# openfheorg/openfhe-boolean-circuit-evaluator

Hardware: AMD Instinct MI355X
Metric: encrypted gate-bootstraps/sec (whole node), AES-128 Bristol ckt STD128 GINX (higher is better)
Workload: dtype u32

## Files before the change

openfhe-boolean-circuit-evaluator_amd/csrc/kernels.hip:

```cpp
#include <hip/hip_runtime.h>

#include <algorithm>
#include <utility>

#include "kernels.hpp"

namespace bce {

#include "phase_prof.hpp"
#include "fused_tail.hpp"
#include "dag_sched.hpp"
#ifdef BCE_PHASE_PROF
__device__ unsigned long long g_phase_prof[BCE_PROF_WAVES * BCE_PROF_SLOTS];
#define BCE_PROF_ARRAY ::bce::g_phase_prof
#endif

__device__ __forceinline__ u32 csub(u32 x, u32 m) { return min(x, x - m); }

__device__ __forceinline__ u32 mul_shoup_lazy(u32 y, uint2 w, u32 Q) {
    u32 qh = __umulhi(w.y, y);
    return w.x * y - qh * Q;
}

__device__ __forceinline__ u64 mad64(u32 a, u32 b, u64 c) {
    u64 r, carry;
    asm("v_mad_u64_u32 %0, %1, %2, %3, %4" : "=v"(r), "=s"(carry) : "v"(a), "v"(b), "v"(c));
    return r;
}
__device__ __forceinline__ u64 mul64(u32 a, u32 b) {
    u64 r, carry;
    asm("v_mad_u64_u32 %0, %1, %2, %3, 0" : "=v"(r), "=s"(carry) : "v"(a), "v"(b));
    return r;
}
__device__ __forceinline__ u32 mul_shoup_lazy3(u32 y, uint2 w, u32 Q) {
    return (u32)mad64(__umulhi(w.y, y), 0u - Q, mul64(y, w.x));
}
__device__ __forceinline__ u64 pair_of(u32 lo) {
    u64 p;
    asm volatile("" : "=v"(p));
    return (p & 0xFFFFFFFF00000000ull) | lo;
}
__device__ __forceinline__ u64 with_lo(u64 pair, u32 lo) { return (pair & 0xFFFFFFFF00000000ull) | lo; }

__device__ __forceinline__ u32 barrett_lazy3(u64 x, u32 Q, u32 shift, u32 mu) {
    return (u32)mad64(__umulhi((u32)(x >> shift), mu), 0u - Q, x);
}

__device__ __forceinline__ u32 barrett_reduce(u64 x, u32 Q, u32 shift, u32 mu) {
    u32 x1 = (u32)(x >> shift);
    u32 qh = __umulhi(x1, mu);
    u32 r = (u32)x - qh * Q;
    r = csub(r, 2 * Q);
    return csub(r, Q);
}

__device__ __forceinline__ u32 barrett_fold(u64 x, u32 c32, u32 Q, u32 shift, u32 mu) {
    return barrett_reduce((u64)(u32)(x >> 32) * c32 + (u32)x, Q, shift, mu);
}

__device__ __forceinline__ u32 phys(u32 j) { return j + ((j >> 6) << 2); }

template <int LOGN>
struct Cfg {
    static constexpr int N = 1 << LOGN;
    static constexpr int LE = LOGN - 6;
    static constexpr int E = 1 << LE;
    static constexpr int NP = N + (N >> 6) * 4;
    static constexpr int F2LO = (6 > LE) ? 6 - LE : 0;
    static_assert(LOGN >= 9 && LOGN <= 11, "supported ring sizes: 512, 1024, 2048");
};

template <u32 M>
__device__ __forceinline__ u32 tw_pos(u32 i) {
    if constexpr (M < 64) {
        return M + i;
    } else {
        constexpr u32 sh = __builtin_ctz(M) - 6;
        return M + ((i & ((1u << sh) - 1u)) << 6) + (i >> sh);
    }
}

__device__ __forceinline__ void block_sync_lds() {
    asm volatile("s_waitcnt lgkmcnt(0)\n\ts_barrier" ::: "memory");
}

__device__ __forceinline__ void wave_sync();
__device__ __forceinline__ void wave_local_sync() {
#ifdef BCE_STEP_BARRIERS
    block_sync_lds();
#else
    wave_sync();
#endif
}
__device__ __forceinline__ void wave_sync() {
    __builtin_amdgcn_fence(__ATOMIC_RELEASE, "wavefront");
    __builtin_amdgcn_wave_barrier();
    __builtin_amdgcn_fence(__ATOMIC_ACQUIRE, "wavefront");
}

template <int LOGN, int LO>
__device__ __forceinline__ u32 elem_j(u32 lane, int r) {
    constexpr int LE = Cfg<LOGN>::LE;
    u32 lane_lo = lane & ((1u << LO) - 1u);
    u32 lane_hi = lane >> LO;
    return (lane_hi << (LO + LE)) | ((u32)r << LO) | lane_lo;
}

template <int LOGN, int LO>
__device__ __forceinline__ void load_pass(const u32* poly, u32 lane, u32 (&x)[Cfg<LOGN>::E]) {
    constexpr int E = Cfg<LOGN>::E;
    if constexpr (LO == 0) {
        const uint4* p = reinterpret_cast<const uint4*>(poly + phys(lane * E));
#pragma unroll
        for (int k = 0; k < E / 4; ++k) {
            uint4 v = p[k];
            x[4 * k] = v.x; x[4 * k + 1] = v.y; x[4 * k + 2] = v.z; x[4 * k + 3] = v.w;
        }
    } else {
#pragma unroll
        for (int r = 0; r < E; ++r) x[r] = poly[phys(elem_j<LOGN, LO>(lane, r))];
    }
}

template <int LOGN, int LO>
__device__ __forceinline__ void store_pass(u32* poly, u32 lane, const u32 (&x)[Cfg<LOGN>::E]) {
    constexpr int E = Cfg<LOGN>::E;
    if constexpr (LO == 0) {
        uint4* p = reinterpret_cast<uint4*>(poly + phys(lane * E));
#pragma unroll
        for (int k = 0; k < E / 4; ++k) p[k] = make_uint4(x[4 * k], x[4 * k + 1], x[4 * k + 2], x[4 * k + 3]);
    } else {
#pragma unroll
        for (int r = 0; r < E; ++r) poly[phys(elem_j<LOGN, LO>(lane, r))] = x[r];
    }
}

template <int LOGN, int LO, int B, bool LAZY>
__device__ __forceinline__ void fwd_stage(u32 (&x)[Cfg<LOGN>::E], u32 lane, const uint2* tw, u32 Q) {
    constexpr int LE = Cfg<LOGN>::LE, E = Cfg<LOGN>::E;
    constexpr int rb = B - LO;
    constexpr u32 m = 1u << (LOGN - 1 - B);
    const u32 hi = (lane >> LO) << (LO + LE - B - 1);
    const u32 Q2 = 2 * Q;
#pragma unroll
    for (int r = 0; r < E; ++r) {
        if (r & (1 << rb)) continue;
        uint2 w = tw[tw_pos<m>(hi | (u32)(r >> (rb + 1)))];
        u32 X = LAZY ? x[r] : csub(x[r], Q2);
        u32 T = mul_shoup_lazy(x[r | (1 << rb)], w, Q);
        x[r] = X + T;
        x[r | (1 << rb)] = X + Q2 - T;
    }
}

template <int LOGN, int LO, int B>
__device__ __forceinline__ void fwd_stage_pair(u64 (&x)[Cfg<LOGN>::E], u32 lane, const uint2* tw, u32 Q) {
    constexpr int LE = Cfg<LOGN>::LE, E = Cfg<LOGN>::E;
    constexpr int rb = B - LO;
    constexpr u32 m = 1u << (LOGN - 1 - B);
    const u32 hi = (lane >> LO) << (LO + LE - B - 1);
    const u32 Q2 = 2 * Q, negQ = 0u - Q;
#pragma unroll
    for (int r = 0; r < E; ++r) {
        if (r & (1 << rb)) continue;
// ... 96 lines not shown
        constexpr int b = gs_bound(r, RB0, RBEND);
        if constexpr (b == 4) x[r] = csub(x[r], 2 * Q);
        else if constexpr (b > 4) x[r] = x[r] - __umulhi(x[r], mu32) * Q;
    };
    (red(std::integral_constant<int, R>{}), ...);
}

template <int LOGN, int LO, int BHI, int BLO, bool LAZY>
__device__ __forceinline__ void fwd_stages(u32 (&x)[Cfg<LOGN>::E], u32 lane, const uint2* tw, u32 Q) {
    if constexpr (BHI >= BLO) {
        fwd_stage<LOGN, LO, BHI, LAZY>(x, lane, tw, Q);
        fwd_stages<LOGN, LO, BHI - 1, BLO, LAZY>(x, lane, tw, Q);
    }
}
template <int LOGN, bool LAZY, bool NORM = true, bool LM_IN = false>
__device__ __forceinline__ void ntt_forward_wave(u32* poly, const uint2* twf, u32 lane, u32 Q, u32 mu32) {
    using C = Cfg<LOGN>;
    u32 x[C::E];
    if constexpr (LAZY && C::F2LO > 0) {
        u64 xp[C::E];
        if constexpr (LM_IN) {
            load_lm<LOGN>(poly, lane, x);
            fwd_first_stage_pair<LOGN>(x, xp, twf[1], Q);
            fwd_stages_pair<LOGN, 6, LOGN - 2, 6>(xp, lane, twf, Q);
        } else {
            load_pass_pair<LOGN, 6>(poly, lane, xp);
            fwd_stages_pair<LOGN, 6, LOGN - 1, 6>(xp, lane, twf, Q);
        }
        store_pass_pair<LOGN, 6>(poly, lane, xp);
        wave_sync();
        load_pass_pair<LOGN, C::F2LO>(poly, lane, xp);
        fwd_stages_pair<LOGN, C::F2LO, 5, C::F2LO>(xp, lane, twf, Q);
        store_pass_pair<LOGN, C::F2LO>(poly, lane, xp);
        wave_sync();
        load_pass<LOGN, 0>(poly, lane, x);
        fwd_stages<LOGN, 0, C::F2LO - 1, 0, LAZY>(x, lane, twf, Q);
    } else {
        if constexpr (LM_IN) load_lm<LOGN>(poly, lane, x);
        else load_pass<LOGN, 6>(poly, lane, x);
        fwd_stages<LOGN, 6, LOGN - 1, 6, LAZY>(x, lane, twf, Q);
        store_pass<LOGN, 6>(poly, lane, x);
        wave_sync();
        load_pass<LOGN, C::F2LO>(poly, lane, x);
        fwd_stages<LOGN, C::F2LO, 5, C::F2LO, LAZY>(x, lane, twf, Q);
        if constexpr (C::F2LO > 0) {
            store_pass<LOGN, C::F2LO>(poly, lane, x);
            wave_sync();
            load_pass<LOGN, 0>(poly, lane, x);
            fwd_stages<LOGN, 0, C::F2LO - 1, 0, LAZY>(x, lane, twf, Q);
        }
    }
    if constexpr (NORM || !LAZY) {
#pragma unroll
        for (int r = 0; r < C::E; ++r) {
            if constexpr (LAZY) {
                u32 v = x[r] - __umulhi(x[r], mu32) * Q;
                x[r] = csub(csub(v, 2 * Q), Q);
            } else {
                x[r] = csub(csub(x[r], 2 * Q), Q);
            }
        }
    }
    store_pass<LOGN, 0>(poly, lane, x);
    wave_sync();
}

__device__ __forceinline__ void ntt_forward_wave_low8(u32* poly, const uint2* twf, u32 lane, u32 Q) {
    constexpr int LOGN = 10;
    {
        u64 xp[16];
        load_pass_pair<LOGN, 4>(poly, lane, xp);
        fwd_stages_pair<LOGN, 4, 7, 4>(xp, lane, twf, Q);
        store_pass_pair<LOGN, 4>(poly, lane, xp);
    }
    wave_sync();
    u32 x[16];
    u64 xp[16];
    load_pass<LOGN, 0>(poly, lane, x);
    fwd_first_stage_pair<LOGN>(x, xp, twf[tw_pos<64>(lane)], Q);
    fwd_stages_pair<LOGN, 0, 2, 0>(xp, lane, twf, Q);
#pragma unroll
    for (int r = 0; r < 16; ++r) x[r] = (u32)xp[r];
    store_pass<LOGN, 0>(poly, lane, x);
    wave_sync();
}
__device__ __forceinline__ void fwd_bfly_pair(u64& xa, u64& xb, uint2 w, u32 Q) {
    const u32 X = (u32)xa, Y = (u32)xb;
    const u64 t = mad64(__umulhi(Y, w.y), 0u - Q, mad64(Y, w.x, xa));
    xb = with_lo(xb, (X << 1) + 2 * Q - (u32)t);
    xa = t;
}
__device__ __forceinline__ void ntt_forward_half_low8(u32* row, u32 h, const uint2* twf, u32 lane, u32 Q) {
    asm volatile("" : "+v"(lane));
    u64 xp[8];
    {
        const u32 l8 = lane >> 5, j0 = (h << 9) | (l8 << 8) | (lane & 31u);
        u32* const p = row + phys(j0);
#pragma unroll
        for (int r = 0; r < 8; ++r) xp[r] = pair_of(p[(r >> 1) * 68 + (r & 1) * 32]);
        const u32 i7 = (h << 1) | l8;
        const uint2 w7 = twf[tw_pos<4>(i7)];
#pragma unroll
        for (int r = 0; r < 4; ++r) fwd_bfly_pair(xp[r], xp[r + 4], w7, Q);
#pragma unroll
        for (int g = 0; g < 2; ++g) {
            const uint2 w6 = twf[tw_pos<8>((i7 << 1) | g)];
            fwd_bfly_pair(xp[4 * g], xp[4 * g + 2], w6, Q);
            fwd_bfly_pair(xp[4 * g + 1], xp[4 * g + 3], w6, Q);
        }
#pragma unroll
        for (int g = 0; g < 4; ++g) fwd_bfly_pair(xp[2 * g], xp[2 * g + 1], twf[tw_pos<16>((i7 << 2) | g)], Q);
#pragma unroll
        for (int r = 0; r < 8; ++r) p[(r >> 1) * 68 + (r & 1) * 32] = (u32)xp[r];
    }
    wave_sync();
    {
        const u32 lh = lane >> 2, j0 = (h << 9) | (lh << 5) | (lane & 3u);
        u32* const p = row + phys(j0);
#pragma unroll
        for (int r = 0; r < 8; ++r) xp[r] = pair_of(p[4 * r]);
        const u32 i4 = (h << 4) | lh;
        const uint2 w4 = twf[tw_pos<32>(i4)];
#pragma unroll
        for (int r = 0; r < 4; ++r) fwd_bfly_pair(xp[r], xp[r + 4], w4, Q);
#pragma unroll
        for (int g = 0; g < 2; ++g) {
            const uint2 w3 = twf[tw_pos<64>((i4 << 1) | g)];
            fwd_bfly_pair(xp[4 * g], xp[4 * g + 2], w3, Q);
            fwd_bfly_pair(xp[4 * g + 1], xp[4 * g + 3], w3, Q);
        }
#pragma unroll
        for (int g = 0; g < 4; ++g) fwd_bfly_pair(xp[2 * g], xp[2 * g + 1], twf[tw_pos<128>((i4 << 2) | g)], Q);
#pragma unroll
        for (int r = 0; r < 8; ++r) p[4 * r] = (u32)xp[r];
    }
    wave_sync();
    {
        const u32 j0 = (h << 9) | (lane << 3);
        uint4* const p = reinterpret_cast<uint4*>(row + phys(j0));
        const uint4 v0 = p[0], v1 = p[1];
        xp[0] = pair_of(v0.x); xp[1] = pair_of(v0.y); xp[2] = pair_of(v0.z); xp[3] = pair_of(v0.w);
        xp[4] = pair_of(v1.x); xp[5] = pair_of(v1.y); xp[6] = pair_of(v1.z); xp[7] = pair_of(v1.w);
        const u32 i1 = (((h << 6) | lane) << 1);
#pragma unroll
        for (int g = 0; g < 2; ++g) {
            const uint2 w1 = twf[tw_pos<256>(i1 | g)];
            fwd_bfly_pair(xp[4 * g], xp[4 * g + 2], w1, Q);
            fwd_bfly_pair(xp[4 * g + 1], xp[4 * g + 3], w1, Q);
        }
#pragma unroll
        for (int g = 0; g < 4; ++g) fwd_bfly_pair(xp[2 * g], xp[2 * g + 1], twf[tw_pos<512>((i1 << 1) | g)], Q);
        p[0] = make_uint4((u32)xp[0], (u32)xp[1], (u32)xp[2], (u32)xp[3]);
        p[1] = make_uint4((u32)xp[4], (u32)xp[5], (u32)xp[6], (u32)xp[7]);
    }
    wave_sync();
}
__device__ __forceinline__ void fwd_bfly(u32& X, u32& Y, uint2 w, u32 Q) {
    const u64 t = mad64(__umulhi(Y, w.y), 0u - Q, mad64(Y, w.x, pair_of(X)));
    Y = (X << 1) + 2 * Q - (u32)t;
    X = (u32)t;
}

template <int LOGN>
__device__ __forceinline__ void ntt_inverse_wave(const u32* src, u32* tmp, const uint2* twi, u32 lane, u32 Q,
                                                 uint2 ninv, uint2 wlast, u32 mu32, u32 (&x)[Cfg<LOGN>::E]) {
    using C = Cfg<LOGN>;
    constexpr int LE = C::LE;
    constexpr auto regs = std::make_integer_sequence<int, C::E>{};
    load_pass<LOGN, 0>(src, lane, x);
    inv_stages<LOGN, 0, 0, LE - 1, 0, false>(x, lane, twi, Q, ninv, wlast);
    inv_pass_reduce<LOGN, 0, LE>(x, Q, mu32, regs);
    store_pass<LOGN, 0>(tmp, lane, x);
    wave_sync();
    load_pass<LOGN, LE>(tmp, lane, x);
    inv_stages<LOGN, LE, LE, 2 * LE - 1, 0, false>(x, lane, twi, Q, ninv, wlast);
    inv_pass_reduce<LOGN, 0, LE>(x, Q, mu32, regs);
    store_pass<LOGN, LE>(tmp, lane, x);
    wave_sync();
    load_pass<LOGN, 6>(tmp, lane, x);
    inv_stages<LOGN, 6, 2 * LE, LOGN - 1, 2 * LE - 6, true>(x, lane, twi, Q, ninv, wlast);
}

template <int LOGN>
__device__ __forceinline__ u32 psi_pow(__amdgpu_buffer_rsrc_t psi_rsrc, u32 e, u32 Q) {
    constexpr u32 N = 1u << LOGN;
    const u32 v = __builtin_amdgcn_raw_buffer_load_b32(psi_rsrc, (e & (N - 1)) << 2, 0, 0);
    return (e & N) ? Q - v : v;
}

__device__ __forceinline__ uint4 bsk_row(__amdgpu_buffer_rsrc_t rsrc, u32 voff, u32 soff) {
    typedef u32 v4u __attribute__((ext_vector_type(4)));
    const v4u v = __builtin_amdgcn_raw_buffer_load_b128(rsrc, voff, soff, 0);
    return make_uint4(v.x, v.y, v.z, v.w);
}


__device__ __forceinline__ u32 gate_const(u32 op, u32 q) {
    u32 e = q >> 3;
    switch (op) {
        case BCE_OR: case BCE_XOR_FAST: return 5 * e;
        case BCE_NOR: case BCE_XNOR_FAST: return e;
        case BCE_NAND: return 3 * e;
        default: return 7 * e;
    }
}

template <int LOGN, bool LAZY, typename PT>
__device__ __forceinline__ void ginx_mac_tail(const PT& P, __amdgpu_buffer_rsrc_t psi_rsrc, u32 Q, u32 ap, uint2 Ia,
                                              uint2 Ina, u32 p0, const u32* accp, u32* accw, const u64 (&sp)[4],
                                              const u64 (&sn)[4], u32 (&a)[4]) {
    constexpr u32 N = 1u << LOGN;
    const bool odd = ap & 1u;
    const u32 k0 = __brev(p0) >> (32 - LOGN);
    const u32 ex = ((2 * k0 + 1) * ap) & (2 * N - 1);
    u32 mp[4], mn[4];
    mp[0] = psi_pow<LOGN>(psi_rsrc, ex, Q);
    mn[0] = psi_pow<LOGN>(psi_rsrc, (2 * N - ex) & (2 * N - 1), Q);
    mp[2] = csub(mul_shoup_lazy(mp[0], Ia, Q), Q);
    mn[2] = csub(mul_shoup_lazy(mn[0], Ina, Q), Q);
    mp[1] = odd ? Q - mp[0] : mp[0];
    mn[1] = odd ? Q - mn[0] : mn[0];
    mp[3] = odd ? Q - mp[2] : mp[2];
    mn[3] = odd ? Q - mn[2] : mn[2];
    const uint4 a4v = *reinterpret_cast<const uint4*>(accp);
    a[0] = a4v.x; a[1] = a4v.y; a[2] = a4v.z; a[3] = a4v.w;
#pragma unroll
    for (int e = 0; e < 4; ++e) {
        if constexpr (LAZY) {
            const u32 rp = barrett_lazy3((u64)(u32)(sp[e] >> 32) * P.c32 + (u32)sp[e], Q, P.red_shift, P.red_mu);
            const u32 rn = barrett_lazy3((u64)(u32)(sn[e] >> 32) * P.c32 + (u32)sn[e], Q, P.red_shift, P.red_mu);
            a[e] = csub(barrett_lazy3((u64)rp * (mp[e] - 1) + (u64)rn * (mn[e] - 1) + a[e], Q, P.red_shift, P.red_mu), 2 * Q);
        } else {
            const u32 rp = barrett_reduce(sp[e], Q, P.red_shift, P.red_mu);
            const u32 rn = barrett_reduce(sn[e], Q, P.red_shift, P.red_mu);
            a[e] = barrett_reduce((u64)rp * (mp[e] - 1) + (u64)rn * (mn[e] - 1) + a[e], Q, P.red_shift, P.red_mu);
        }
    }
    *reinterpret_cast<uint4*>(accw) = make_uint4(a[0], a[1], a[2], a[3]);
}

__device__ __forceinline__ u32 redc(u64 x, u32 Q, u32 qn) { return (u32)(mad64((u32)x * qn, Q, x) >> 32); }
template <int LOGN, typename PT>
__device__ __forceinline__ void ginx_mac_tail_redc(const PT& P, __amdgpu_buffer_rsrc_t psi_r2_rsrc, u32 Q, u32 ap, uint2 Ia,
                                                   uint2 Ina, u32 p0, const u32* accp, u32* accw, const u64 (&sp)[4],
                                                   const u64 (&sn)[4], u32 (&a)[4]) {
    constexpr u32 N = 1u << LOGN;
    const bool odd = ap & 1u;
    const u32 k0 = __brev(p0) >> (32 - LOGN);
    const u32 ex = ((2 * k0 + 1) * ap) & (2 * N - 1);
    const u32 off = P.r2_off, K = Q + 2 * off, qn = P.qinv_neg;
    u32 mp[4], mn[4];
    const u32 p0r = psi_pow<LOGN>(psi_r2_rsrc, ex, Q), n0r = psi_pow<LOGN>(psi_r2_rsrc, (2 * N - ex) & (2 * N - 1), Q);
    mp[0] = p0r + off;
    mn[0] = n0r + off;
    mp[2] = csub(mul_shoup_lazy(p0r, Ia, Q), Q) + off;
    mn[2] = csub(mul_shoup_lazy(n0r, Ina, Q), Q) + off;
    mp[1] = odd ? K - mp[0] : mp[0];
    mn[1] = odd ? K - mn[0] : mn[0];
    mp[3] = odd ? K - mp[2] : mp[2];
    mn[3] = odd ? K - mn[2] : mn[2];
    const uint4 a4v = *reinterpret_cast<const uint4*>(accp);
    a[0] = a4v.x; a[1] = a4v.y; a[2] = a4v.z; a[3] = a4v.w;
#pragma unroll
    for (int e = 0; e < 4; ++e) {
        const u32 rp = redc(sp[e], Q, qn), rn = redc(sn[e], Q, qn);
        a[e] = csub(redc(mad64(rn, mn[e], mul64(rp, mp[e])), Q, qn) + a[e], 2 * Q);
    }
    *reinterpret_cast<uint4*>(accw) = make_uint4(a[0], a[1], a[2], a[3]);
}

template <int LOGN, bool LAZY, u32 T, typename PT>
__device__ __forceinline__ void bootstrap_prologue(const PT& P, const bce_gate_desc& g, u32 soff, uint2* twf, u32* acc,
                                                   u32* av, u32 tid, u32 lane, u32 wave) {
    using C = Cfg<LOGN>;
    constexpr int N = C::N, NP = C::NP;
    const u32 Q = P.Q, q = P.q, qm = q - 1, n = P.n;
    for (u32 i = tid; i < (u32)N; i += T) twf[i] = P.tw_f[i];
    {
        const u32* in0 = P.pool + (size_t)(g.in0 + soff) * P.pool_stride;
        const u32* in1 = P.pool + (size_t)(g.in1 + soff) * P.pool_stride;
        const bool two = g.op <= BCE_XNOR_FAST;
        for (u32 i = tid; i <= n; i += T) {
            u32 v0 = in0[i];
            if (g.neg0) v0 = ((i == n ? (q >> 2) : 0u) - v0) & qm;
            u32 v = v0;
            if (two) {
                u32 v1 = in1[i];
                if (g.neg1) v1 = ((i == n ? (q >> 2) : 0u) - v1) & qm;
                v = (g.op == BCE_XOR_FAST || g.op == BCE_XNOR_FAST) ? (2u * (v0 - v1)) & qm : (v0 + v1) & qm;
            } else if (i == n) {
                v = (v0 + (q >> 2)) & qm;
            }
            av[i] = v;
        }
    }
    __syncthreads();
    {
        const u32 b = av[n];
        const u32 q1 = gate_const(g.op, q), q2 = (q1 + (q >> 1)) & qm;
        const u32 pos = P.Q8p1, neg = Q - P.Q8p1;
        for (u32 j = tid; j < (u32)N; j += T) {
            u32 v = 0;
            if (j % P.factor == 0) {
                u32 t = (b - j / P.factor) & qm;
                bool in = (q1 < q2) ? (t >= q1 && t < q2) : !(t >= q2 && t < q1);
                v = in ? neg : pos;
// ... 189 lines not shown
        u32* out = acc_out + ((size_t)blockIdx.x * 2 + wave) * N;
#pragma unroll
        for (int r = 0; r < E; ++r) out[((u32)r << 6) | lane] = x[r];
    }
}

__device__ __forceinline__ u32 xlay1(u32 p) { return (p & 15u) + 20u * ((p >> 4) & 3u) + 80u * ((p >> 6) & 3u) + 320u * (p >> 8); }
__device__ __forceinline__ u32 xlay2(u32 p) { return (p & 63u) + 80u * ((p >> 6) & 3u) + 320u * (p >> 8); }

__device__ __forceinline__ void inv_pass4(u32 (&x)[4], uint2 fa, uint2 fb, uint2 fc, u32 Q, u32 mu32) {
    const u32 Q2 = 2 * Q;
    const u32 a0 = x[0] + x[1];
    const u32 a1 = mul_shoup_lazy3(x[1] + Q2 - x[0], fa, Q);
    const u32 a2 = x[2] + x[3];
    const u32 a3 = mul_shoup_lazy3(x[3] + Q2 - x[2], fb, Q);
    const u32 b0 = a0 + a2;
    x[2] = mul_shoup_lazy3(a2 + 2 * Q2 - a0, fc, Q);
    const u32 b1 = a1 + a3;
    x[3] = mul_shoup_lazy3(a3 + Q2 - a1, fc, Q);
    x[0] = b0 - __umulhi(b0, mu32) * Q;
    x[1] = csub(b1, Q2);
}
__device__ __forceinline__ void inv_pass4_last(u32 (&x)[4], uint2 fa, uint2 fb, uint2 ninv, uint2 wlast, u32 Q) {
    const u32 Q2 = 2 * Q;
    const u32 a0 = x[0] + x[1];
    const u32 a1 = mul_shoup_lazy3(x[1] + Q2 - x[0], fa, Q);
    const u32 a2 = x[2] + x[3];
    const u32 a3 = mul_shoup_lazy3(x[3] + Q2 - x[2], fb, Q);
    x[0] = csub(mul_shoup_lazy3(a0 + a2, ninv, Q), Q);
    x[2] = csub(mul_shoup_lazy3(a0 + 2 * Q2 - a2, wlast, Q), Q);
    x[1] = csub(mul_shoup_lazy3(a1 + a3, ninv, Q), Q);
    x[3] = csub(mul_shoup_lazy3(a1 + Q2 - a3, wlast, Q), Q);
}

template <bool REGTW>
struct SplitInv {
    u32 a0, x0, l1, s1, l2, s2, l3, s3, t;
    uint2 fa[REGTW ? 5 : 1], fb[REGTW ? 5 : 1], fc[REGTW ? 4 : 1];
    u32 ia[REGTW ? 1 : 4], ic[REGTW ? 1 : 4];
};
template <bool REGTW>
__device__ __forceinline__ void split_inv_setup(SplitInv<REGTW>& S, const uint2* twf, u32 t) {
    S.t = t;
    S.a0 = phys(4 * t);
    const u32 wb = 48u * (t >> 6);
    S.x0 = S.a0 + wb;
    const u32 pb1 = ((t >> 2) << 4) | (t & 3u), pb2 = ((t >> 4) << 6) | (t & 15u), pb3 = ((t >> 6) << 8) | (t & 63u);
    S.l1 = phys(pb1) + wb; S.s1 = xlay1(pb1);
    S.l2 = xlay1(pb2); S.s2 = xlay2(pb2);
    S.l3 = xlay2(pb3); S.s3 = 320u * (t >> 6) + (t & 63u);
    const u32 u0 = t, u1 = t >> 2, u2 = t >> 4, u3 = t >> 6;
    if constexpr (REGTW) {
        S.fa[0] = twf[tw_pos<512>(511 - 2 * u0)]; S.fb[0] = twf[tw_pos<512>(510 - 2 * u0)]; S.fc[0] = twf[tw_pos<256>(255 - u0)];
        S.fa[1] = twf[tw_pos<128>(127 - 2 * u1)]; S.fb[1] = twf[tw_pos<128>(126 - 2 * u1)]; S.fc[1] = twf[tw_pos<64>(63 - u1)];
        S.fa[2] = twf[tw_pos<32>(31 - 2 * u2)];   S.fb[2] = twf[tw_pos<32>(30 - 2 * u2)];   S.fc[2] = twf[tw_pos<16>(15 - u2)];
        S.fa[3] = twf[tw_pos<8>(7 - 2 * u3)];     S.fb[3] = twf[tw_pos<8>(6 - 2 * u3)];     S.fc[3] = twf[tw_pos<4>(3 - u3)];
        S.fa[4] = twf[tw_pos<2>(1)];              S.fb[4] = twf[tw_pos<2>(0)];
    } else {
        S.ia[0] = tw_pos<512>(511 - 2 * u0); S.ic[0] = tw_pos<256>(255 - u0);
        S.ia[1] = tw_pos<128>(127 - 2 * u1); S.ic[1] = tw_pos<64>(63 - u1);
        S.ia[2] = tw_pos<32>(31 - 2 * u2);   S.ic[2] = tw_pos<16>(15 - u2);
        S.ia[3] = tw_pos<8>(7 - 2 * u3);     S.ic[3] = tw_pos<4>(3 - u3);
    }
}
template <bool REGTW, int K>
__device__ __forceinline__ void split_tw(const SplitInv<REGTW>& S, const uint2* twf, uint2& fa, uint2& fb, uint2& fc) {
    if constexpr (REGTW) { fa = S.fa[K]; fb = S.fb[K]; fc = S.fc[K]; }
    else {
        constexpr u32 M = 512u >> (2 * K);
        fa = twf[S.ia[K]];
        fb = twf[M < 64 ? S.ia[K] - 1 : S.ia[K] - 64];
        fc = twf[S.ic[K]];
    }
}
template <bool REGTW>
__device__ __forceinline__ void split_pass0(const SplitInv<REGTW>& S, const uint2* twf, u32 (&a)[4], u32* xa, u32 Q, u32 mu32) {
    uint2 fa, fb, fc;
    split_tw<REGTW, 0>(S, twf, fa, fb, fc);
    inv_pass4(a, fa, fb, fc, Q, mu32);
    *reinterpret_cast<uint4*>(xa + S.x0) = make_uint4(a[0], a[1], a[2], a[3]);
}
template <bool REGTW, typename F>
__device__ __forceinline__ void split_inverse_rest(const SplitInv<REGTW>& S, const uint2* twf, u32* xa, u32* xb, u32 Q, u32 mu32,
                                                   uint2 ninv, uint2 wlast, u32 (&x)[4], F&& at_pass) {
    uint2 fa, fb, fc;
    wave_sync();
    at_pass(std::integral_constant<int, 1>{});
#pragma unroll
    for (int r = 0; r < 4; ++r) x[r] = xa[S.l1 + 4 * r];
    split_tw<REGTW, 1>(S, twf, fa, fb, fc);
    inv_pass4(x, fa, fb, fc, Q, mu32);
#pragma unroll
    for (int r = 0; r < 4; ++r) xb[S.s1 + 4 * r] = x[r];
    wave_local_sync();
    at_pass(std::integral_constant<int, 2>{});
#pragma unroll
    for (int r = 0; r < 4; ++r) x[r] = xb[S.l2 + 20 * r];
    split_tw<REGTW, 2>(S, twf, fa, fb, fc);
    inv_pass4(x, fa, fb, fc, Q, mu32);
#pragma unroll
    for (int r = 0; r < 4; ++r) xa[S.s2 + 16 * r] = x[r];
    wave_local_sync();
    at_pass(std::integral_constant<int, 3>{});
#pragma unroll
    for (int r = 0; r < 4; ++r) x[r] = xa[S.l3 + 80 * r];
    split_tw<REGTW, 3>(S, twf, fa, fb, fc);
    inv_pass4(x, fa, fb, fc, Q, mu32);
#pragma unroll
    for (int r = 0; r < 4; ++r) xb[S.s3 + 64 * r] = x[r];
    block_sync_lds();
    at_pass(std::integral_constant<int, 4>{});
#pragma unroll
    for (int r = 0; r < 4; ++r) x[r] = xb[S.t + 320 * r];
    if constexpr (REGTW) inv_pass4_last(x, S.fa[4], S.fb[4], ninv, wlast, Q);
    else inv_pass4_last(x, twf[tw_pos<2>(1)], twf[tw_pos<2>(0)], ninv, wlast, Q);
}

template <int DG, int WPS, bool AP, bool FUSE, bool FOLD, bool PERSIST = false, typename PT>
__device__ __forceinline__ void lat_bootstrap(const PT& P, const bce_gate_desc g, const u32 soff, const u32 boot, u32* smem,
                                              u32* __restrict__ acc_out, u32* __restrict__ dbg_lweN, u32* __restrict__ dbg_ks) {
    static_assert(DG == 4, "the split inverse transform is laid out for 8 waves");
    constexpr int LOGN = 10;
    using C = Cfg<LOGN>;
    constexpr int N = C::N, NP = C::NP;
    constexpr u32 R = 2 * DG, T = 64 * R, XB = 1280;
    uint2* twf = reinterpret_cast<uint2*>(smem);
    u32* acc = reinterpret_cast<u32*>(twf + N);
    u32* dct = acc + 2 * NP;
    u32* xab = dct + R * NP;
    u32* av = xab + 4 * XB;

    u32 tid_ = threadIdx.x;
    if constexpr (PERSIST) asm volatile("" : "+v"(tid_));
    const u32 tid = tid_;
    const u32 lane = tid & 63;
    const u32 wave = __builtin_amdgcn_readfirstlane(tid >> 6);
    const u32 Q = P.Q, q = P.q, qm = q - 1, n = P.n;
    if constexpr (WPS >= 4 && !PERSIST) {
        if (P.xcd_gate != nullptr && wave == 0) {
            const u32 xcc = __builtin_amdgcn_s_getreg((31u << 11) | 20u) & 15u;
            u32* const gate = P.xcd_gate + 32u * xcc;
            const u32 slots = max(2u, 2u * (P.cu_count >> 3));
            const u32 mine = (gridDim.x + 7u - xcc) >> 3;
            const u32 t = u_add(gate, 1u);
            const u32 full = (t / slots + 1u) * slots, target = full < mine ? full : mine;
            const u64 t0 = __builtin_amdgcn_s_memrealtime();
            while (u_ld(gate) < target && __builtin_amdgcn_s_memrealtime() - t0 < P.xcd_gate_ticks) __builtin_amdgcn_s_sleep(8);
        }
    }
    bootstrap_prologue<LOGN, true, T>(P, g, soff, twf, acc, av, tid, lane, wave);

    const u32 c = wave >> 2;
    constexpr bool REGTW = WPS <= 2;
    SplitInv<REGTW> S;
    split_inv_setup(S, twf, tid & 255u);
    u32* const accc = acc + c * NP;
    u32* const xa = xab + c * 2 * XB;
    u32* const xb = xa + XB;

    const uint2 ninv = make_uint2(P.Ninv, P.Ninv_s), wlast = make_uint2(P.Winv_last, P.Winv_last_s);
    constexpr u32 rgsw = R * 2 * N;
    const __amdgpu_buffer_rsrc_t rsrc =
        __builtin_amdgcn_make_buffer_rsrc(const_cast<u32*>(P.bsk), 0, AP ? 0x7FFFFFFF : (int)(n * 2 * rgsw * 4), 0x00020000);
#ifdef BCE_BARRETT_TAIL
    const __amdgpu_buffer_rsrc_t psi_rsrc = __builtin_amdgcn_make_buffer_rsrc(const_cast<u32*>(P.psi_tab), 0, N * 4, 0x00020000);
#else
    const __amdgpu_buffer_rsrc_t psi_rsrc = __builtin_amdgcn_make_buffer_rsrc(const_cast<u32*>(P.psi_tab_r2), 0, N * 4, 0x00020000);
#endif
    const u32 gb = P.gBits, Qh = Q >> 1;
    u32 off = 0;
    for (u32 l = 0; l < (u32)DG; ++l) off |= 1u << (l * gb + gb - 1);
    const u32 offm = off - Q, bias = Q - (1u << (gb - 1));
    const u32 mc = tid / (N / 4), mp0 = (tid % (N / 4)) * 4, mpp = phys(mp0);
    const u32 dig0 = phys(S.t);
    const uint2 w9 = twf[1], w8a = twf[2], w8b = twf[3];
    {
        const uint4 v = *reinterpret_cast<const uint4*>(accc + S.a0);
        u32 a[4] = {v.x, v.y, v.z, v.w};
        split_pass0(S, twf, a, xa, Q, P.mu32);
    }

    BCE_PROF_INIT();
    const u32 nsteps = AP ? n * P.dR : n;
    u32 cb = 0;
    if constexpr (WPS >= 4) __builtin_amdgcn_s_setprio(2);
    for (u32 step = 0; step < nsteps; ++step) {
        u32 ap = 0, rowb;
        if constexpr (!AP) {
            ap = ((q - av[step]) & qm) * P.factor;
            if (ap == 0) continue;
            rowb = step * (2 * rgsw * 4);
        } else {
            const u32 i = step / P.dR, kd = step - i * P.dR;
            u32 aI = (q - av[i]) & qm;
            for (u32 t = 0; t < kd; ++t) aI /= P.baseR;
            const u32 a0 = aI % P.baseR;
            if (a0 == 0) continue;
            rowb = (((i * P.baseR + a0) * P.dR + kd) * rgsw) * 4u;
        }
        constexpr u32 PR = (WPS <= 2) ? R : R / 2;
        uint4 kA[R], kB[R];
        auto request_rows = [&](auto kc) {
            constexpr u32 k = decltype(kc)::value - 1, G = PR / 4;
            BCE_PROF_MARK(8 + k);
#pragma unroll
            for (u32 l = k * G; l < (k + 1) * G; ++l) {
                kA[l] = bsk_row(rsrc, tid * 16u, rowb + l * (2 * N * 4));
                if constexpr (!AP) kB[l] = bsk_row(rsrc, tid * 16u, rowb + (rgsw + l * 2 * N) * 4);
            }
        };
        {
            u32 x[4], u[4];
            split_inverse_rest(S, twf, xa, xb, Q, P.mu32, ninv, wlast, x, request_rows);
#pragma unroll
            for (int r = 0; r < 4; ++r) u[r] = x[r] + ((x[r] < Qh) ? off : offm);
#pragma unroll
            for (u32 l = FOLD ? 1 : 0; l < (u32)DG; ++l) {
                u32 v[4];
#pragma unroll
                for (int r = 0; r < 4; ++r) v[r] = __builtin_amdgcn_ubfe(u[r], l * gb, gb) + bias;
                fwd_bfly(v[0], v[2], w9, Q);
                fwd_bfly(v[1], v[3], w9, Q);
                fwd_bfly(v[0], v[1], w8a, Q);
                fwd_bfly(v[2], v[3], w8b, Q);
#pragma unroll
                for (int r = 0; r < 4; ++r) dct[(2 * l + c) * NP + dig0 + 272 * r] = v[r];
            }
        }
        BCE_PROF_MARK(0);
        block_sync_lds();
        BCE_PROF_MARK(1);
        if constexpr (WPS >= 4) { if (FOLD && wave >= 4) __builtin_amdgcn_s_setprio(1); else __builtin_amdgcn_s_setprio(0); }
#ifndef BCE_SKIP_FWD
        if constexpr (FOLD) {
            if (wave < 4) ntt_forward_wave_low8(dct + (2 + wave) * NP, twf, lane, Q);
            else ntt_forward_half_low8(dct + (6 + ((wave - 4) >> 1)) * NP, (wave - 4) & 1u, twf, lane, Q);
        } else {
            ntt_forward_wave_low8(dct + wave * NP, twf, lane, Q);
        }
#endif
        if constexpr (WPS >= 4) __builtin_amdgcn_s_setprio(2);
        BCE_PROF_MARK(2);
        if constexpr (PR < R) {
#pragma unroll
            for (u32 l = PR; l < R; ++l) kA[l] = bsk_row(rsrc, tid * 16u, rowb + l * (2 * N * 4));
#pragma unroll
            for (u32 l = PR; l < R; ++l) if constexpr (!AP) kB[l] = bsk_row(rsrc, tid * 16u, rowb + (rgsw + l * 2 * N) * 4);
        }
        block_sync_lds();
        BCE_PROF_MARK(3);
        {
            u64 sp[4] = {0, 0, 0, 0}, sn[4] = {0, 0, 0, 0};
#pragma unroll
            for (u32 l = 0; l < R; ++l) {
#ifdef BCE_SKIP_MAC
                const uint4 d = make_uint4(l + tid, l, tid, 1u);
#else
                const uint4 d = *reinterpret_cast<const uint4*>((FOLD && l < 2 ? acc + cb : dct) + l * NP + mpp);
#endif
                sp[0] += (u64)d.x * kA[l].x; sp[1] += (u64)d.y * kA[l].y; sp[2] += (u64)d.z * kA[l].z; sp[3] += (u64)d.w * kA[l].w;
                if constexpr (!AP) {
                    sn[0] += (u64)d.x * kB[l].x; sn[1] += (u64)d.y * kB[l].y; sn[2] += (u64)d.z * kB[l].z; sn[3] += (u64)d.w * kB[l].w;
                }
            }
            u32 anew[4];
            const u32* const accr = acc + cb + mc * NP + mpp;
            u32* const accw = acc + (FOLD ? 2 * NP - cb : 0) + mc * NP + mpp;
            if constexpr (AP) {
#pragma unroll
                for (int e = 0; e < 4; ++e) anew[e] = barrett_fold(sp[e], P.c32, Q, P.red_shift, P.red_mu);
                *reinterpret_cast<uint4*>(accw) = make_uint4(anew[0], anew[1], anew[2], anew[3]);
            } else {
                const u32 a4 = ap & 3u;
                const uint2 Ia = make_uint2(P.I4[a4], P.I4s[a4]);
                const uint2 Ina = make_uint2(P.I4[(4u - a4) & 3u], P.I4s[(4u - a4) & 3u]);
#ifdef BCE_BARRETT_TAIL
                ginx_mac_tail<LOGN, true>(P, psi_rsrc, Q, ap, Ia, Ina, mp0, accr, accw, sp, sn, anew);
#else
                ginx_mac_tail_redc<LOGN>(P, psi_rsrc, Q, ap, Ia, Ina, mp0, accr, accw, sp, sn, anew);
#endif
            }
            if constexpr (FOLD) cb = 2 * NP - cb;
            split_pass0(S, twf, anew, xa, Q, P.mu32);
        }
        BCE_PROF_MARK(4);
        wave_local_sync();
        BCE_PROF_MARK(5);
    }
    BCE_PROF_FLUSH();
    {
        u32 x[4];
        split_inverse_rest(S, twf, xa, xb, Q, P.mu32, ninv, wlast, x, [](auto) {});
        if (acc_out) {
            u32* out = acc_out + ((size_t)boot * 2 + c) * N + S.t;
#pragma unroll
            for (int r = 0; r < 4; ++r) out[256 * r] = x[r];
        }
        if constexpr (FUSE) {
#pragma unroll
            for (int r = 0; r < 4; ++r) acc[c * N + S.t + 256 * r] = x[r];
        }
    }
    if constexpr (FUSE) {
        if constexpr (WPS >= 4) __builtin_amdgcn_s_setprio(0);
        __syncthreads();
        u32* rowidx = dct;
        u64* red = reinterpret_cast<u64*>(dct + ((N * P.dKS + 3) & ~3u));
        u32* outp = P.pool + (size_t)(g.out + soff) * P.pool_stride;
        if (P.ksk_u16) fused_tail<uint16_t, T>(P, acc, rowidx, red, outp, boot, dbg_lweN, dbg_ks);
        else fused_tail<u32, T>(P, acc, rowidx, red, outp, boot, dbg_lweN, dbg_ks);
    }
}

template <int DG, int WPS, bool AP = false, bool FUSE = false, bool FOLD = false>
__global__ __launch_bounds__(128 * DG, WPS) void k_blind_rotate_lat(DevParams P, const bce_gate_desc* __restrict__ descs, u32 n_desc,
                                                                   u32 slot_stride, u32* __restrict__ acc_out,
                                                                   u32* __restrict__ dbg_lweN, u32* __restrict__ dbg_ks) {
    extern __shared__ __align__(16) u32 smem[];
    lat_bootstrap<DG, WPS, AP, FUSE, FOLD>(P, descs[blockIdx.x % n_desc], (blockIdx.x / n_desc) * slot_stride, blockIdx.x, smem,
                                           acc_out, dbg_lweN, dbg_ks);
}

bool fused_tail_fits(const DevParams& P) {
    const size_t N = P.N, NP = N + (N >> 6) * 4, R = 2 * P.dG;
    const size_t VW = P.ksk_u16 ? 8 : 4, G = (P.n + VW) / VW, Gv = G < 512 ? G : 512, RW = (Gv + 63) / 64, SL = 8 / RW;
    const size_t need = ((N * P.dKS + 3) & ~(size_t)3) * 4 + SL * Gv * VW * 8;
    return (size_t)P.n + 1 <= 512 * VW && RW <= 8 && need <= (R * NP + 4 * 1280) * 4;
}

size_t blind_rotate_lat_lds_bytes(const DevParams& P) {
    const size_t N = P.N, NP = N + (N >> 6) * 4, R = 2 * P.dG;
    return (2 * N + (2 + R) * NP + 4 * 1280 + ((P.n + 1 + 3) & ~3u)) * sizeof(u32);
}

size_t blind_rotate_lds_bytes(const DevParams& P) {
    const size_t N = P.N, NP = N + (N >> 6) * 4, R = 2 * P.dG;
    return (2 * N + (2 + R) * NP + ((P.n + 1 + 3) & ~3u)) * sizeof(u32);
}

__global__ void k_dag_rearm(DagParams D) {
    const size_t stride = (size_t)gridDim.x * blockDim.x, i0 = (size_t)blockIdx.x * blockDim.x + threadIdx.x;
    const size_t items = (size_t)D.n_tasks * D.instances;
    for (size_t i = i0; i < items; i += stride) D.dep[i] = D.dep_init[i % D.n_tasks];
    for (u32 q = 0; q < kDagQueues; ++q) {
        const u32 ninit = (D.init_off[q + 1] - D.init_off[q]) * D.instances;
        for (size_t j = i0; j < D.qcap[q]; j += stride) {
            u32 v = 0;
            if (j < ninit) {
                const u32 ti = (u32)(j / D.instances), k = (u32)(j % D.instances);
                v = k * D.n_tasks + D.init_items[D.init_off[q] + ti] + 1u;
            }
            D.slots[q][j] = v;
        }
        if (i0 == 0) { D.ctl[q] = 0; D.ctl[kDagQueues + q] = ninit; D.ctl[kDagIdleCus] = 0; }
    }
    for (size_t j = i0 + kDagAbort; j < kDagCtlWords; j += stride) D.ctl[j] = 0;
}

template <int WPS, bool AP, bool FOLD>
__global__ __launch_bounds__(512, WPS) void k_bootstrap_dag(const DevParams* Pp, const DagParams* Dp) {
    extern __shared__ __align__(16) u32 smem[];
    dag_worker(Dp, smem, [&](ConstDagParams& D, u32 t, u32 k) {
        lat_bootstrap<4, WPS, AP, true, FOLD, true>(*as_constant<ConstDevParams>(Pp), D.tasks[t], D.slot_base + k * D.slot_stride, 0,
                                                   smem + kDagMailboxWords, nullptr, nullptr, nullptr);
    });
}

bool dag_kernel_available(const DevParams& P) {
    if (P.is64) return dag64_kernel_available(P);
    return !P.is64 && P.variant != 1 && P.logN == 10 && P.dG == 4 && P.lazy && fused_tail_fits(P);
}

hipError_t launch_dag_rearm(const DagParams& D, hipStream_t s) {
    hipLaunchKernelGGL(k_dag_rearm, dim3(1024), dim3(256), 0, s, D);
    return hipGetLastError();
}

hipError_t launch_bootstrap_dag(const DevParams& P, const DevParams* d_P, const DagParams* d_params, int wps, u32 grid, hipStream_t s) {
    if (!dag_kernel_available(P)) return hipErrorInvalidValue;
    if (P.is64) return launch_bootstrap_dag64(P, d_P, d_params, grid, s);
    using DagKernel = void (*)(const DevParams*, const DagParams*);
    const bool ap = P.method_ap != 0, x1 = wps <= 2;
    DagKernel k;
    if (P.fold) k = ap ? (x1 ? k_bootstrap_dag<2, true, true> : k_bootstrap_dag<4, true, true>) : (x1 ? k_bootstrap_dag<2, false, true> : k_bootstrap_dag<4, false, true>);
    else k = ap ? (x1 ? k_bootstrap_dag<2, true, false> : k_bootstrap_dag<4, true, false>) : (x1 ? k_bootstrap_dag<2, false, false> : k_bootstrap_dag<4, false, false>);
    const size_t lds = blind_rotate_lat_lds_bytes(P) + kDagMailboxWords * 4;
    hipError_t e = hipFuncSetAttribute(reinterpret_cast<const void*>(k), hipFuncAttributeMaxDynamicSharedMemorySize, (int)lds);
// ... 387 lines not shown
```

Baseline: 156,200.

## Split folded forward NTT into per-wave quarter slices across three rows

Adds a forward-NTT variant in which each wave processes one quarter of three polynomial rows at once, so all eight waves carry equal work instead of four doing full rows and four doing half rows. It uses permlane16/32 swaps for cross-lane butterfly exchanges in place of some LDS round trips, and drops the priority split that favoured the half-row waves. It is enabled by default through a macro. The cost is higher register pressure (twelve 64-bit values per lane) and a different LDS access pattern that may introduce bank conflicts.

```diff
diff --git a/openfhe-boolean-circuit-evaluator_amd/csrc/kernels.hip b/openfhe-boolean-circuit-evaluator_amd/csrc/kernels.hip
--- a/openfhe-boolean-circuit-evaluator_amd/csrc/kernels.hip
+++ b/openfhe-boolean-circuit-evaluator_amd/csrc/kernels.hip
@@ -10,6 +10,9 @@
 #include "phase_prof.hpp"
 #include "fused_tail.hpp"
 #include "dag_sched.hpp"
+#ifndef BCE_FWD_QUARTERS
+#define BCE_FWD_QUARTERS 1
+#endif
 #ifdef BCE_PHASE_PROF
 __device__ unsigned long long g_phase_prof[BCE_PROF_WAVES * BCE_PROF_SLOTS];
 #define BCE_PROF_ARRAY ::bce::g_phase_prof
@@ -412,6 +415,98 @@
         for (int g = 0; g < 4; ++g) fwd_bfly_pair(xp[2 * g], xp[2 * g + 1], twf[tw_pos<512>((i1 << 1) | g)], Q);
         p[0] = make_uint4((u32)xp[0], (u32)xp[1], (u32)xp[2], (u32)xp[3]);
         p[1] = make_uint4((u32)xp[4], (u32)xp[5], (u32)xp[6], (u32)xp[7]);
+    }
+    wave_sync();
+}
+__device__ __forceinline__ void swap_lane5(u64& a, u64& b) {
+    const auto r = __builtin_amdgcn_permlane32_swap((u32)a, (u32)b, false, false);
+    a = pair_of(r[0]);
+    b = pair_of(r[1]);
+}
+__device__ __forceinline__ void swap_lane4(u64& a, u64& b) {
+    const auto r = __builtin_amdgcn_permlane16_swap((u32)a, (u32)b, false, false);
+    a = pair_of(r[0]);
+    b = pair_of(r[1]);
+}
+__device__ __forceinline__ void ntt_forward_quarters_low8(u32* rows, u32 g, const uint2* twf, u32 lane, u32 Q) {
+    constexpr u32 NP = Cfg<10>::NP;
+    asm volatile("" : "+v"(lane));
+    u32* const q0 = rows + 272u * g;
+    u64 xp[3][4];
+    {
+        u32* const p = q0 + lane;
+#pragma unroll
+        for (int s = 0; s < 3; ++s)
+#pragma unroll
+            for (int r = 0; r < 4; ++r) xp[s][r] = pair_of(p[s * NP + 68 * r]);
+        const uint2 w7 = twf[tw_pos<4>(g)], w6a = twf[tw_pos<8>(2 * g)], w6b = twf[tw_pos<8>(2 * g + 1)];
+#pragma unroll
+        for (int s = 0; s < 3; ++s) {
+            fwd_bfly_pair(xp[s][0], xp[s][2], w7, Q);
+            fwd_bfly_pair(xp[s][1], xp[s][3], w7, Q);
+            fwd_bfly_pair(xp[s][0], xp[s][1], w6a, Q);
+            fwd_bfly_pair(xp[s][2], xp[s][3], w6b, Q);
+            swap_lane5(xp[s][0], xp[s][2]);
+            swap_lane5(xp[s][1], xp[s][3]);
+            swap_lane4(xp[s][0], xp[s][1]);
+            swap_lane4(xp[s][2], xp[s][3]);
+        }
+    }
+    {
+        const u32 lh = lane >> 4, ll = lane & 15u;
+        const uint2 w5 = twf[tw_pos<16>((g << 2) | lh)];
+        const uint2 w4a = twf[tw_pos<32>((g << 3) | (lh << 1))], w4b = twf[tw_pos<32>((g << 3) | (lh << 1) | 1u)];
+#pragma unroll
+        for (int s = 0; s < 3; ++s) {
+            fwd_bfly_pair(xp[s][0], xp[s][2], w5, Q);
+            fwd_bfly_pair(xp[s][1], xp[s][3], w5, Q);
+            fwd_bfly_pair(xp[s][0], xp[s][1], w4a, Q);
+            fwd_bfly_pair(xp[s][2], xp[s][3], w4b, Q);
+        }
+        u32* const p = q0 + 68u * lh + ll;
+#pragma unroll
+        for (int s = 0; s < 3; ++s)
+#pragma unroll
+            for (int r = 0; r < 4; ++r) p[s * NP + 16 * r] = (u32)xp[s][r];
+    }
+    wave_sync();
+    const u32 m = lane & 15u, pm = 16u * m + 4u * (m >> 2);
+    {
+        const u32 t = lane >> 4;
+        u32* const p = q0 + pm + t;
+#pragma unroll
+        for (int s = 0; s < 3; ++s)
+#pragma unroll
+            for (int r = 0; r < 4; ++r) xp[s][r] = pair_of(p[s * NP + 4 * r]);
+        const u32 i3 = (g << 4) | m;
+        const uint2 w3 = twf[tw_pos<64>(i3)], w2a = twf[tw_pos<128>(i3 << 1)], w2b = twf[tw_pos<128>((i3 << 1) | 1u)];
+#pragma unroll
+        for (int s = 0; s < 3; ++s) {
+            fwd_bfly_pair(xp[s][0], xp[s][2], w3, Q);
+            fwd_bfly_pair(xp[s][1], xp[s][3], w3, Q);
+            fwd_bfly_pair(xp[s][0], xp[s][1], w2a, Q);
+            fwd_bfly_pair(xp[s][2], xp[s][3], w2b, Q);
+            swap_lane5(xp[s][0], xp[s][2]);
+            swap_lane5(xp[s][1], xp[s][3]);
+            swap_lane4(xp[s][0], xp[s][1]);
+            swap_lane4(xp[s][2], xp[s][3]);
+        }
+    }
+    {
+        const u32 t = lane >> 4;
+        const u32 i1 = (g << 6) | (m << 2) | t;
+        const uint2 w1 = twf[tw_pos<256>(i1)], w0a = twf[tw_pos<512>(i1 << 1)], w0b = twf[tw_pos<512>((i1 << 1) | 1u)];
+#pragma unroll
+        for (int s = 0; s < 3; ++s) {
+            fwd_bfly_pair(xp[s][0], xp[s][2], w1, Q);
+            fwd_bfly_pair(xp[s][1], xp[s][3], w1, Q);
+            fwd_bfly_pair(xp[s][0], xp[s][1], w0a, Q);
+            fwd_bfly_pair(xp[s][2], xp[s][3], w0b, Q);
+        }
+        u32* const p = q0 + pm + 4u * t;
+#pragma unroll
+        for (int s = 0; s < 3; ++s)
+            *reinterpret_cast<uint4*>(p + s * NP) = make_uint4((u32)xp[s][0], (u32)xp[s][1], (u32)xp[s][2], (u32)xp[s][3]);
     }
     wave_sync();
 }
@@ -907,6 +1002,7 @@
 
     const u32 c = wave >> 2;
     constexpr bool REGTW = WPS <= 2;
+    constexpr bool FWDQ = BCE_FWD_QUARTERS != 0;
     SplitInv<REGTW> S;
     split_inv_setup(S, twf, tid & 255u);
     u32* const accc = acc + c * NP;
@@ -985,9 +1081,11 @@
         BCE_PROF_MARK(0);
         block_sync_lds();
         BCE_PROF_MARK(1);
-        if constexpr (WPS >= 4) { if (FOLD && wave >= 4) __builtin_amdgcn_s_setprio(1); else __builtin_amdgcn_s_setprio(0); }
+        if constexpr (WPS >= 4) { if (FOLD && !FWDQ && wave >= 4) __builtin_amdgcn_s_setprio(1); else __builtin_amdgcn_s_setprio(0); }
 #ifndef BCE_SKIP_FWD
-        if constexpr (FOLD) {
+        if constexpr (FOLD && FWDQ) {
+            ntt_forward_quarters_low8(dct + (2 + 3 * (wave >> 2)) * NP, wave & 3u, twf, lane, Q);
+        } else if constexpr (FOLD) {
             if (wave < 4) ntt_forward_wave_low8(dct + (2 + wave) * NP, twf, lane, Q);
             else ntt_forward_half_low8(dct + (6 + ((wave - 4) >> 1)) * NP, (wave - 4) & 1u, twf, lane, Q);
         } else {
```

After: 156,300, median of 6. Within noise of the previous version (+0.1%).
